# HagesLab/Bayesian-Inference-TRPL

Measured on AMD Instinct MI355X. Metric: TRPL timesteps/sec at 128 nodes (system = parameter sample x excitation; fused solve + log-likelihood; parameter-sample likelihoods/sec in likelihoods_per_s_*), higher is better.
Workload: dtype f64

## Files before the change

### bayesian-inference-trpl_amd/csrc/stepper_pair_impl.hpp

```cpp
#pragma once
#include "stepper_impl.hpp"

namespace trpl {
TRPL_VARIANT_NS_BEGIN
namespace pair {

constexpr int L = 128;
constexpr int NR = 4;
constexpr int WS = 32;

__device__ __forceinline__ double lane_value(double v, int l)
{
    return __hiloint2double(__builtin_amdgcn_readlane(__double2hiint(v), l),
                            __builtin_amdgcn_readlane(__double2loint(v), l));
}

__device__ __forceinline__ void half_sums(double v, double &lo, double &hi)
{
    v = dpp_add<0x111, 0xF>(v);
    v = dpp_add<0x112, 0xF>(v);
    v = dpp_add<0x114, 0xF>(v);
    v = dpp_add<0x118, 0xF>(v);
    v = dpp_add<0x142, 0xA>(v);
    lo = lane_value(v, 31);
    hi = lane_value(v, 63);
}

struct Terms2 {
    double q;
    unsigned long long neg, nonneg;
};
__device__ __forceinline__ Terms2 no_terms2() { return {0.0, 0ull, ~0ull}; }

// ... 39 lines not shown
        }
    }
    if (reductions) (*reductions)++;
    double sA, sB;
    half_sums(t.q, sA, sB);
    okA = sA < 0.0;
    okB = sB < 0.0;
}

template <bool ISO>
__device__ __forceinline__ void update_field2(const MatPar &m, double a0, const double (&Nk)[NR], const double (&Pk)[NR],
                                              const double (&bE)[NR], double (&Ek)[NR], int lane, bool act)
{
    double Nm[NR], Pm[NR], A[NR], b[NR], rA[NR];
    nbrB_dn<double, NR, 1>(Nk, Nm, lane);
    nbrB_dn<double, NR, 1>(Pk, Pm, lane);
    if constexpr (ISO) {
        const bool first = (lane & (WS - 1)) == 0;
        Nm[0] = first ? 0.0 : Nm[0];
        Pm[0] = first ? 0.0 : Pm[0];
    }
#pragma unroll
    for (int j = 0; j < NR; j++) {
        A[j] = __builtin_fma(m.hLDP, Pk[j] + Pm[j], __builtin_fma(m.hLDN, Nk[j] + Nm[j], a0));
        b[j] = __builtin_fma(m.LDP, Pk[j] - Pm[j], __builtin_fma(-m.LDN, Nk[j] - Nm[j], -bE[j]));
    }
    rcp_rows<NR>(A, rA);
    const bool act0 = act && (lane & (WS - 1)) != 0;
    Ek[0] = act0 ? b[0] * rA[0] : Ek[0];
#pragma unroll
    for (int j = 1; j < NR; j++) Ek[j] = act ? b[j] * rA[j] : Ek[j];
}

template <bool ISO, bool SNAP = false, bool OPT = (TRPL_PAIR_OPTIMISTIC != 0)>
__global__ void __launch_bounds__(64, 2) stepper_pair_kernel(const StepArgs a)
{
    constexpr int LAY = 2;
    const int lane = threadIdx.x;
    const int ln = lane & (WS - 1);
    const bool hi = lane >= WS;
    const int64_t blk = blockIdx.x;
    int cA = (int)(blk % a.C), cB = cA;
    int64_t sA = 2 * (blk / a.C), sB = sA + 1;
    if (a.pair_n > 0) {
        const int k = cA;
        cA = a.pair_cA[k]; cB = a.pair_cB[k];
        sB = sA + a.pair_oB[k];
        sA = sA + a.pair_oA[k];
        if (sA >= a.S) return;
    }
    const bool validB = sB < a.S;
    if (!validB) { sB = sA; cB = cA; }
    const int64_t s = hi ? sB : sA;
    const int c = hi ? cB : cA;
    const CurveConst &cc = a.curve[cA];

    const double *xs = a.X + s * a.xld;
    const double N0 = xs[0] * cc.scales[0], P0 = xs[1] * cc.scales[1], DN = xs[2] * cc.scales[2],
                 DP = xs[3] * cc.scales[3], rate = xs[4] * cc.scales[4], sr0 = xs[5] * cc.scales[5],
                 srL = xs[6] * cc.scales[6], CN = xs[7] * cc.scales[7], CP = xs[8] * cc.scales[8],
                 tauN = xs[9] * cc.scales[9], tauP = xs[10] * cc.scales[10],
                 Lambda = xs[11] * cc.scales[11];
    const double n0p0 = N0 * P0;
    MatPar mp_ = {N0, P0, DN, DP, rate, sr0, srL, CN, CP, tauN, tauP, Lambda, n0p0,
                  ln == 0 ? 1.0 : 0.0, ln == WS - 1 ? 1.0 : 0.0};
    mp_.fast_constants();
    mp_.boundary_constants();
    MatPar mp = mp_;
    const double mag = a.xld > 12 ? xs[12] : 0.0;
    const double TOL = a.TOL;
    const int MAX = a.MAX;
    constexpr bool PREDICT = TRPL_STEPPER_PREDICT != 0;

    constexpr int HSLOT = 2 * NR * 64;
    constexpr bool MOMENTS = TRPL_STEPPER_MOMENTS != 0;
    constexpr bool WEIGHTED = TRPL_STEPPER_WEIGHTED != 0;
    constexpr bool CUT = TRPL_STEPPER_CUT != 0;
    constexpr bool PARKED = MOMENTS || CUT;
    static_assert(!CUT || !SNAP, "the cut sink exists in likelihood mode only");
    __shared__ __attribute__((aligned(16))) double lds[4 * HSLOT + (PARKED ? 6 : 0)];
    double2 *hist2 = reinterpret_cast<double2 *>(lds);
    double *xch = nullptr;
    double Nk[NR], Pk[NR], Ek[NR], hE[4][NR];
#pragma unroll
    for (int j = 0; j < NR; j++) {
        const double raw = (SNAP && a.resN != nullptr) ? 0.0 : a.dN[(int64_t)c * L + NR * ln + j];
        const double dn = raw * cc.dx3;
        Nk[j] = N0 + dn;
        Pk[j] = P0 + dn;
        Ek[j] = 0.0;
#pragma unroll
        for (int m = 0; m < 4; m++) {
            hE[m][j] = 0.0;
            hist2[(m * NR + j) * 64 + lane] = make_double2(0.0, 0.0);
        }
    }

    PlSinkT<MOMENTS, PARKED, WEIGHTED, CUT> sinkA(a, cc, cA, sA, lane_value(mag, 0));
    PlSinkT<MOMENTS, PARKED, WEIGHTED, CUT> sinkB(a, cc, cB, sB, lane_value(mag, WS));
    const double rateA = lane_value(rate, 0), rateB = lane_value(rate, WS);
    if constexpr (PARKED) { sinkA.set_park(lds + 4 * HSLOT); sinkB.set_park(lds + 4 * HSLOT + 3); }
    sinkA.set_floor(rateA, lane_value(n0p0, 0), L);
    sinkB.set_floor(rateB, lane_value(n0p0, WS), L);
    int statusA = 0, statusB = 0;
    bool deadA = false, deadB = !validB;
    int64_t itotA = 0, itotB = 0;
#if TRPL_VOTE_STATS
    int nredN = 0, nredP = 0;
#define TRPL_STAT(x) &x
#else
#define TRPL_STAT(x) nullptr
#endif
    SnapSink snap(a, cc);
    auto park = [&](bool mine) {
        if (mine) {
            MatPar b_ = {1.0, 1.0, 1.0, 1.0, 0.0, 0.0, 0.0, 0.0, 0.0, 1.0, 1.0, 0.0, 1.0,
                         ln == 0 ? 1.0 : 0.0, ln == WS - 1 ? 1.0 : 0.0};
            b_.fast_constants();
            b_.boundary_constants();
            mp = b_;
        }
#pragma unroll
        for (int j = 0; j < NR; j++) {
            if (mine) {
                Nk[j] = 1.0; Pk[j] = 1.0; Ek[j] = 0.0;
#pragma unroll
                for (int m = 0; m < 4; m++) {
                    hE[m][j] = 0.0;
                    hist2[(m * NR + j) * 64 + lane] = make_double2(1.0, 1.0);
                }
            }
        }
    };

    int32_t t_begin = 0;
    if constexpr (SNAP) {
        if (a.resN != nullptr) {
            t_begin = (int32_t)a.t0;
            const int64_t r5 = (hi ? sinkB.orow : sinkA.orow) * 5;
#pragma unroll
            for (int j = 0; j < NR; j++) {
                const int i = NR * ln + j;
                Nk[j] = a.resN[(r5 + 4) * L + i]; Pk[j] = a.resP[(r5 + 4) * L + i]; Ek[j] = a.resE[(r5 + 4) * (L + 1) + i];
#pragma unroll
                for (int m = 0; m < 4; m++) {
                    const int slot = (int)((a.t0 - 1 - m) & 3);
                    const double e_ = a.resE[(r5 + 3 - m) * (L + 1) + i];
                    hE[m][j] = e_;
                    hist2[(slot * NR + j) * 64 + lane] = make_double2(a.resN[(r5 + 3 - m) * L + i], a.resP[(r5 + 3 - m) * L + i]);
                }
            }
            statusA = status_of_checkpoint(a.resN[(sinkA.orow * 5 + 4) * L], a.t0);
            statusB = validB ? status_of_checkpoint(a.resN[(sinkB.orow * 5 + 4) * L], a.t0) : 0;
            deadA = statusA != 0;
            deadB = deadB || statusB != 0;
            if (statusA || statusB) park(hi ? statusB != 0 : statusA != 0);
        }
    }
    int32_t pl_next = 0, pl_col = 0;
    if constexpr (SNAP) {
        if (t_begin > 0) { pl_col = (t_begin + a.plT - 1) / a.plT; pl_next = pl_col * a.plT; sinkA.base = sinkB.base = pl_col; }
    }
    const int32_t row_cap = bdf_row_cap(a.flags);
    for (int32_t t = t_begin; t <= sinkA.t_last; t++) {
        if (deadA && deadB) break;
        if constexpr (SNAP) {
            if (snap.due(t))
                snap.template take<NR, L>(Nk, Pk, Ek, hi ? sinkB.orow : sinkA.orow, hi ? !deadB : !deadA,
                                          [&](int j) { return NR * ln + j; });
        }
        double a0, a1, a2, a3, a4, a5;
        bdf_row<double>(t < row_cap ? t : row_cap, a0, a1, a2, a3, a4, a5);

        double plA = 0.0, plB = 0.0;
        const bool pl_step = t == pl_next;
        if (pl_step) {
            double q = __builtin_fma(Nk[0], Pk[0], -n0p0);
#pragma unroll
            for (int j = 1; j < NR; j++) q += __builtin_fma(Nk[j], Pk[j], -n0p0);
            double hA, hB;
            half_sums(q, hA, hB);
            plA = rateA * hA;
            plB = rateB * hB;
        }

        double bN[NR], bP[NR], bE[NR];
        {
            const int s1 = (int)((t + 3) & 3) * NR, s2 = (int)((t + 2) & 3) * NR,
                      s3 = (int)((t + 1) & 3) * NR, s4 = (int)(t & 3) * NR;
#pragma unroll
            for (int j = 0; j < NR; j++) {
                const double2 h1 = hist2[(s1 + j) * 64 + lane], h2 = hist2[(s2 + j) * 64 + lane],
                              h3 = hist2[(s3 + j) * 64 + lane], h4 = hist2[(s4 + j) * 64 + lane];
                bN[j] = a1 * Nk[j] + a2 * h1.x + a3 * h2.x + a4 * h3.x + a5 * h4.x;
                bP[j] = a1 * Pk[j] + a2 * h1.y + a3 * h2.y + a4 * h3.y + a5 * h4.y;
                hist2[(s4 + j) * 64 + lane] = make_double2(Nk[j], Pk[j]);
                if constexpr (PREDICT) {
                    Nk[j] = predict_start(Nk[j], h1.x, h2.x, t);
                    Pk[j] = predict_start(Pk[j], h1.y, h2.y, t);
                }
            }
#pragma unroll
            for (int j = 0; j < NR; j++) {
                bE[j] = a1 * Ek[j] + a2 * hE[0][j] + a3 * hE[1][j] + a4 * hE[2][j] + a5 * hE[3][j];
#pragma unroll
                for (int m = 3; m >= 1; m--) hE[m][j] = hE[m - 1][j];
                hE[0][j] = Ek[j];
                if constexpr (PREDICT) Ek[j] = predict_start(Ek[j], hE[1][j], hE[2][j], t);
            }
        }

        bool doneA = deadA, doneB = deadB;
        int itA = MAX, itB = MAX;
        auto iterate_once = [&](auto frozen_c, auto seam_c, int iters) {
            constexpr bool FROZEN = decltype(frozen_c)::value;
            constexpr bool SEAM = decltype(seam_c)::value;
            const bool act = FROZEN ? (hi ? !doneB : !doneA) : true;
            double lo_[NR], dg[NR], up[NR], bb[NR], Ep[NR], x[NR];
            nbrB_up<double, NR, 1>(Ek, Ep, lane);
            bool okNA, okNB, okPA, okPB;
            const bool needNA = FROZEN ? !doneA : true, needNB = FROZEN ? !doneB : true;
            assemble<LAY, true, NR, WS, L, true>(mp, a0, Nk, Pk, Ek, Ep, bN, lo_, dg, up, bb, ln);
            const Terms2 tN = residual_terms2<SEAM>(lo_, dg, up, bb, Nk, TOL, lane);
            residual_verdict2(tN, needNA, needNB, okNA, okNB, TRPL_STAT(nredN));
            cr_pcr_solve<double, NR, WS, SEAM, true>(lo_, dg, up, bb, x, lane, xch);
#pragma unroll
            for (int j = 0; j < NR; j++) Nk[j] = act ? x[j] : Nk[j];
            assemble<LAY, false, NR, WS, L, true>(mp, a0, Nk, Pk, Ek, Ep, bP, lo_, dg, up, bb, ln);
            const bool needPA = needNA && okNA, needPB = needNB && okNB;
            Terms2 tP = no_terms2();
            if (needPA || needPB) {
                tP = residual_terms2<SEAM>(lo_, dg, up, bb, Pk, TOL, lane);
                residual_verdict2(tP, needPA, needPB, okPA, okPB, TRPL_STAT(nredP));
            } else {
                okPA = okPB = false;
            }
            cr_pcr_solve<double, NR, WS, SEAM, true>(lo_, dg, up, bb, x, lane, xch);
#pragma unroll
            for (int j = 0; j < NR; j++) Pk[j] = act ? x[j] : Pk[j];
            update_field2<ISO>(mp, a0, Nk, Pk, bE, Ek, lane, act);
            if (!doneA && okNA && okPA) { doneA = true; itA = iters + 1; }
            if (!doneB && okNB && okPB) { doneB = true; itB = iters + 1; }
        };
        auto iterate_step = [&](auto seam_c) {
            int iters = 0;
            for (; iters < MAX && !(doneA || doneB); iters++) iterate_once(std::false_type{}, seam_c, iters);
            for (; iters < MAX && !(doneA && doneB); iters++) iterate_once(std::true_type{}, seam_c, iters);
        };
        if constexpr (ISO && OPT) {
            iterate_step(std::false_type{});
            static_assert(NR % 4 == 0, "the witness relies on rcp_rows taking ONE reciprocal of the product of a lane's rows (pcr.hpp)");
            const double wit = Ek[NR - 1];
            const bool finite2 = TRPL_PAIR_WITNESS == 0 || __builtin_amdgcn_ballot_w64(__builtin_isfinite(wit)) == ~0ull;
            if ((!deadA && itA >= MAX) || (!deadB && itB >= MAX) || !finite2) {
                const int s4 = (int)(t & 3) * NR;
#pragma unroll
                for (int j = 0; j < NR; j++) {
                    const double2 h = hist2[(s4 + j) * 64 + lane];
                    if constexpr (PREDICT) {
                        const double2 h1 = hist2[((int)((t + 3) & 3) * NR + j) * 64 + lane],
                                      h2 = hist2[((int)((t + 2) & 3) * NR + j) * 64 + lane];
                        Nk[j] = predict_start(h.x, h1.x, h2.x, t);
                        Pk[j] = predict_start(h.y, h1.y, h2.y, t);
                        Ek[j] = predict_start(hE[0][j], hE[1][j], hE[2][j], t);
                    } else {
                        Nk[j] = h.x; Pk[j] = h.y; Ek[j] = hE[0][j];
                    }
                }
                doneA = deadA; doneB = deadB; itA = itB = MAX;
                iterate_step(std::true_type{});
            }
        } else {
            iterate_step(std::integral_constant<bool, ISO>{});
        }
        bool killA = false, killB = false;
        if (!deadA) { itotA += itA; if (itA >= MAX) { statusA = 1 + (int)t; killA = true; } }
        if (!deadB) { itotB += itB; if (itB >= MAX) { statusB = 1 + (int)t; killB = true; } }
        if (killA || killB) {
            park(hi ? killB : killA);
            deadA = deadA || killA;
            deadB = deadB || killB;
        }

        if (pl_step) {
            if (!deadA) sinkA.push(pl_col, plA);
            if (!deadB) sinkB.push(pl_col, plB);
            pl_next += a.plT;
            pl_col++;
            if constexpr (CUT) {
                if ((pl_col & 63) == 0) {
                    const bool cutA = !deadA && sinkA.is_cut(), cutB = !deadB && sinkB.is_cut();
                    if (cutA || cutB) {
                        park(hi ? cutB : cutA);
                        deadA = deadA || cutA;
                        deadB = deadB || cutB;
                    }
                }
            }
        }

    }

    {
        const int64_t doneA_ = statusA ? (int64_t)(statusA - 1) : sinkA.t_last + 1;
        const int64_t doneB_ = statusB ? (int64_t)(statusB - 1) : sinkB.t_last + 1;
        sinkA.flush_batch((int)((doneA_ + a.plT - 1) / a.plT - sinkA.base));
        if (validB) sinkB.flush_batch((int)((doneB_ + a.plT - 1) / a.plT - sinkB.base));
    }
    if constexpr (SNAP) {
        if (statusA && !hi) snap.template fail_fill<L>(sinkA.orow, statusA, ln, WS);
        if (statusB && hi && validB) snap.template fail_fill<L>(sinkB.orow, statusB, ln, WS);
    }
#if TRPL_VOTE_STATS
    itotA += ((int64_t)nredN << 24) + ((int64_t)nredP << 44);
#endif
    sinkA.finish(statusA, itotA);
    if (validB) sinkB.finish(statusB, itotB);
#undef TRPL_STAT
}

}

template <bool ISO>
hipError_t launch_stepper_pair_t(const StepArgs &a, hipStream_t stream)
{
    if (a.L != pair::L) return hipErrorInvalidValue;
    const int64_t nblk = ((a.S + 1) / 2) * a.C;
    if (nblk <= 0) return hipSuccess;
    const bool always_seam = (a.flags & kFlagPairAlwaysSeam) != 0;
    const bool snap = a.n_snap > 0 || a.resN != nullptr;
    const dim3 grid((unsigned)nblk), block(64);
#if TRPL_STEPPER_MOMENTS || TRPL_STEPPER_CUT
    if (snap || !sink_args_ok(a)) return hipErrorInvalidValue;
    if (always_seam) hipLaunchKernelGGL((pair::stepper_pair_kernel<ISO, false, false>), grid, block, 0, stream, a);
    else             hipLaunchKernelGGL((pair::stepper_pair_kernel<ISO, false>), grid, block, 0, stream, a);
#else
    if (always_seam) {
        if (snap) hipLaunchKernelGGL((pair::stepper_pair_kernel<ISO, true, false>), grid, block, 0, stream, a);
        else      hipLaunchKernelGGL((pair::stepper_pair_kernel<ISO, false, false>), grid, block, 0, stream, a);
    } else {
        if (snap) hipLaunchKernelGGL((pair::stepper_pair_kernel<ISO, true>), grid, block, 0, stream, a);
        else      hipLaunchKernelGGL((pair::stepper_pair_kernel<ISO, false>), grid, block, 0, stream, a);
    }
#endif
    return hipGetLastError();
}
TRPL_VARIANT_NS_END

}
```

### bayesian-inference-trpl_amd/csrc/trpl_api.hip

```cpp
#include <hip/hip_runtime.h>
#include <dlfcn.h>
#include <math.h>
#include <stdarg.h>
#include <stdio.h>
#include <stdlib.h>
#include <string.h>

#include <algorithm>
#include <chrono>
#include <vector>

#include "api_util.hpp"
#include "crosslane.hpp"

namespace trpl {

namespace { thread_local char g_err[512] = ""; }

int api_fail(int code, const char *fmt, ...)
{
    va_list ap;
    va_start(ap, fmt);
    vsnprintf(g_err, sizeof g_err, fmt, ap);
    va_end(ap);
// ... 298 lines not shown

static int no_cut_flag(uint32_t flags)
{
    if (flags & TRPL_FLAG_CUT)
        return api_fail(TRPL_ERR_ARG, "TRPL_FLAG_CUT is set by trpl_loglik_cut[_dev] only: this entry point has no sse_cut");
    return TRPL_OK;
}

int no_weighted_flag(uint32_t flags)
{
    if (int rc = no_cut_flag(flags)) return rc;
    if (flags & TRPL_FLAG_WEIGHTED)
        return api_fail(TRPL_ERR_ARG, "TRPL_FLAG_WEIGHTED is set by trpl_loglik_weighted[_dev] only: this entry point takes no weights");
    return TRPL_OK;
}

int no_moments_flag(uint32_t flags)
{
    if (int rc = no_weighted_flag(flags)) return rc;
    if (flags & TRPL_FLAG_MOMENTS)
        return api_fail(TRPL_ERR_ARG, "TRPL_FLAG_MOMENTS is set by trpl_loglik_moments[_dev] only: this entry point has no esum output");
    return TRPL_OK;
}

int select_device(int32_t device)
{
    int n = 0;
    if (hipGetDeviceCount(&n) != hipSuccess || n <= 0) return api_fail(TRPL_ERR_NODEVICE, "no HIP device visible");
    if (device < 0 || device >= n) return api_fail(TRPL_ERR_ARG, "device %d out of range (%d visible)", device, n);
    HIP_TRY(hipSetDevice(device));
    return TRPL_OK;
}

}

using namespace trpl;

namespace {

int launch(const trpl::StepArgs &a_in, uint32_t flags, hipStream_t st, int64_t steps)
{
    if (int rc = check_launch(flags, a_in.L, steps, a_in.n_snap > 0, a_in.resN != nullptr)) return rc;
    const StepperChoice c = classify_stepper(flags, a_in.L, a_in.S * a_in.C, steps, a_in.n_snap > 0 || a_in.resN != nullptr);
    trpl::StepArgs a = a_in;
    a.bundle = c.bundle;
    if (c.family == StepperChoice::Pair) build_pair_table(a);
    static const char *const kWord[trpl::Variant::kUnits] = {"", "", "pair ", "fp32 ", "mixed ", "hist32 "};
    StepperLauncher *const fn = find_launcher(c);
    if (!fn) return api_fail(TRPL_ERR_UNSUPPORTED, "no stepper is built for this combination of flags (flags 0x%x, L = %d)", flags, a.L);
    const hipError_t e = fn(a, st);
    if (e != hipSuccess) return api_fail(TRPL_ERR_HIP, "%sstepper launch: %s", kWord[unit_of(c)], hipGetErrorString(e));
    return TRPL_OK;
}

}

extern "C" {

int trpl_abi_version(void) { return TRPL_ABI_VERSION; }
int trpl_has_experimental(void)
{
#ifdef TRPL_EXPERIMENTAL
    return 1;
#else
    return 0;
#endif
}
const char *trpl_last_error(void) { return g_err; }

int trpl_kernel_variant(int64_t nsys, int32_t L, int64_t steps, uint32_t flags)
{
    const StepperChoice c = classify_stepper(flags, L, nsys, steps, false);
    if (c.family == StepperChoice::F32) return TRPL_KERNEL_FP32;
    if (c.strict) return TRPL_KERNEL_STRICT;
    if (c.mixed) return TRPL_KERNEL_MIXED;
    if (c.hist32) return TRPL_KERNEL_HIST32;
    return c.family == StepperChoice::Pair ? TRPL_KERNEL_FAST_PAIR : TRPL_KERNEL_FAST;
}

int trpl_kernel_name(int64_t nsys, int32_t L, int64_t steps, uint32_t flags, int32_t snapshots, char *buf, int64_t buflen)
{
    if (!buf || buflen < 1) return api_fail(TRPL_ERR_ARG, "buf must hold at least one byte");
    buf[0] = 0;
    if (int rc = check_launch(flags, L, steps, snapshots != 0 && !(flags & TRPL_FLAG_FP32), false)) return rc;
    const StepperChoice c = classify_stepper(flags, L, nsys, steps, snapshots != 0);
    if (!find_launcher(c)) return api_fail(TRPL_ERR_UNSUPPORTED, "no stepper is built for this combination of flags (flags 0x%x, L = %d)", flags, L);
    const char *tf[2] = {"false", "true"};
    char ns[64];
    snprintf(ns, sizeof ns, "trpl::%s%s", kSinks[c.sink].ns, c.predict ? "predict::" : "");
    int n;
    if (c.family == StepperChoice::F32)
        n = snprintf(buf, (size_t)buflen, "%sf32::stepper_kernel<%d>", ns, c.L);
    else if (c.family == StepperChoice::Pair)
        n = snprintf(buf, (size_t)buflen, "%spair::stepper_pair_kernel<true, %s, %s>", ns, tf[c.snap], tf[c.optimistic]);
    else
        n = snprintf(buf, (size_t)buflen, "%sstepper_kernel<%d, %s, %s, %s, %s, %s>", ns, c.L, tf[c.strict], tf[c.snap],
                     tf[c.mixed], tf[c.bundle > 1], tf[c.hist32]);
    if (n < 0 || n >= buflen) return api_fail(TRPL_ERR_ARG, "buflen=%lld is too small for the kernel name", (long long)buflen);
    return TRPL_OK;
}

// ... 1075 lines not shown
```

### bayesian-inference-trpl_amd/csrc/trpl_common.hpp

```cpp
#pragma once
#include <hip/hip_runtime.h>
#include <stdint.h>

namespace trpl {

constexpr int kMaxCurves = 16;
constexpr int kMaxSnaps = 16;
constexpr int kMaxBundle = 16;
__host__ __device__ constexpr int bundle_cap(int L) { return L <= 64 ? 16 : 4; }

struct CurveConst {
    double scales[12];
    double dx3;
    double plnorm;
    double dx;
    int64_t n_obs;
};

struct StepArgs {
    const double *X;
    const double *dN;
    const double *obs;
    const int32_t *obs_hi;
    const double *obs_dx;
    const double *obs_h;
    void *pl;
    double *sse;
    int32_t *status;
    int64_t *iters_total;
    int32_t *floor_col;
    double *snapN, *snapP, *snapE;
    const double *resN, *resP, *resE;
    int64_t t0;
    int64_t S;
    int64_t T;
    int64_t pl_ld;
    int64_t obs_ld;
    double TOL;
    int32_t xld;
    int32_t C;
    int32_t L;
    int32_t plT;
    int32_t MAX;
    int32_t pl_bytes;
    uint32_t flags;
    int32_t bundle;
    int32_t n_snap;
    int32_t snap_ld;
    int32_t snap_t[kMaxSnaps];
    int32_t snap_slot[kMaxSnaps];
    int32_t pair_n;
    uint8_t pair_cA[kMaxCurves], pair_oA[kMaxCurves], pair_cB[kMaxCurves], pair_oB[kMaxCurves];
    CurveConst curve[kMaxCurves];
    double *esum;
    const double *wts;
    double sse_cut;
    int32_t *cut_col;
    const double *cut_level;
};

__host__ __device__ constexpr uint32_t flags_bdf_order(uint32_t flags) { return (flags >> 14) & 7u; }
__host__ __device__ constexpr int32_t bdf_row_cap(uint32_t flags) { return flags_bdf_order(flags) ? (int32_t)flags_bdf_order(flags) - 1 : 4; }
constexpr int32_t flags_bundle(uint32_t flags) { return (int32_t)((flags >> 8) & 0xFu) + 1; }
template <typename T>
__device__ __forceinline__ void bdf_row(int32_t row, T &a0, T &a1, T &a2, T &a3, T &a4, T &a5)
{
    if (row == 0)      { a0 = (T)1.0; a1 = (T)-1.0; a2 = (T)0.0; a3 = (T)0.0; a4 = (T)0.0; a5 = (T)0.0; }
    else if (row == 1) { a0 = (T)1.5; a1 = (T)-2.0; a2 = (T)0.5; a3 = (T)0.0; a4 = (T)0.0; a5 = (T)0.0; }
    else if (row == 2) { a0 = (T)(11.0 / 6); a1 = (T)-3.0; a2 = (T)1.5; a3 = (T)(-1.0 / 3); a4 = (T)0.0; a5 = (T)0.0; }
    else if (row == 3) { a0 = (T)(25.0 / 12); a1 = (T)-4.0; a2 = (T)3.0; a3 = (T)(-4.0 / 3); a4 = (T)0.25; a5 = (T)0.0; }
    else               { a0 = (T)(137.0 / 60); a1 = (T)-5.0; a2 = (T)5.0; a3 = (T)(-10.0 / 3); a4 = (T)1.25; a5 = (T)-0.2; }
}

void interp_rows_any(const void *pl, int elem_bytes, int64_t rows, int64_t ld, const int32_t *hi, const double *dx,
                     const double *h, int64_t n_obs, double *out, int64_t out_ld);
struct Variant {
    enum Sink { plain, moments, weighted, cut, kSinks };
    enum Unit { fast, strict, pair, f32, mixed, hist32, kUnits };
};
template <int SINK, int PREDICT, int UNIT> hipError_t launch_variant(const StepArgs &a, hipStream_t stream);
#define TRPL_VARIANT(sink, predict, unit) \
    template <> hipError_t launch_variant<Variant::sink, predict, Variant::unit>(const StepArgs &a, hipStream_t stream);
#include "stepper_variants.hpp"
#undef TRPL_VARIANT

hipError_t launch_log10_clamp(void *x, int elem_bytes, int64_t rows, int64_t cols, int64_t ld, double mn,
                              hipStream_t stream);
hipError_t launch_sse_accumulate(double *P, const void *pl, int elem_bytes, int64_t rows, int64_t n_obs,
                                 int64_t ld, const double *values, const double *mag, hipStream_t stream);
hipError_t launch_reduce_curves(double *P, const double *sse, int64_t S, int C, hipStream_t stream);
hipError_t launch_budget_level(const double *budget, const double *sse, double *cut_level, int64_t S, int c0, int g, hipStream_t stream);
hipError_t launch_pl_loglik(const void *pl, int elem_bytes, int64_t rows, int64_t ld, const double *obs,
// ... 39 lines not shown
```

Baseline: 616.4 million.

## Make pair stepper persistent with atomic ticket work distribution

Wraps the pair stepper kernel body in a loop so a resident-sized grid of blocks pulls pair work items from a global atomic ticket counter instead of launching one block per pair. Ticket slots are tracked on the host with events so they can be reused across launches, and a fallback to the classic launch exists when no slot is free. This is meant to balance the uneven per-pair iteration counts and reduce block scheduling tail. The cost is atomic traffic, extra host bookkeeping, and risk around slot reuse and counter reset.

```diff
diff --git a/bayesian-inference-trpl_amd/csrc/stepper_pair_impl.hpp b/bayesian-inference-trpl_amd/csrc/stepper_pair_impl.hpp
--- a/bayesian-inference-trpl_amd/csrc/stepper_pair_impl.hpp
+++ b/bayesian-inference-trpl_amd/csrc/stepper_pair_impl.hpp
@@ -1,4 +1,7 @@
 #pragma once
+#include <atomic>
+#include <mutex>
+
 #include "stepper_impl.hpp"
 
 namespace trpl {
@@ -104,291 +107,405 @@
     for (int j = 1; j < NR; j++) Ek[j] = act ? b[j] * rA[j] : Ek[j];
 }
 
+template <bool SNAP>
+constexpr bool kPersistent = !SNAP && TRPL_STEPPER_PREDICT == 0;
+
+struct Ticket { unsigned next, done; };
+constexpr int kLiveSlots = 32;
+static __device__ Ticket g_ticket[kLiveSlots];
+
 template <bool ISO, bool SNAP = false, bool OPT = (TRPL_PAIR_OPTIMISTIC != 0)>
 __global__ void __launch_bounds__(64, 2) stepper_pair_kernel(const StepArgs a)
 {
-    constexpr int LAY = 2;
-    const int lane = threadIdx.x;
-    const int ln = lane & (WS - 1);
-    const bool hi = lane >= WS;
-    const int64_t blk = blockIdx.x;
-    int cA = (int)(blk % a.C), cB = cA;
-    int64_t sA = 2 * (blk / a.C), sB = sA + 1;
-    if (a.pair_n > 0) {
-        const int k = cA;
-        cA = a.pair_cA[k]; cB = a.pair_cB[k];
-        sB = sA + a.pair_oB[k];
-        sA = sA + a.pair_oA[k];
-        if (sA >= a.S) return;
-    }
-    const bool validB = sB < a.S;
-    if (!validB) { sB = sA; cB = cA; }
-    const int64_t s = hi ? sB : sA;
-    const int c = hi ? cB : cA;
-    const CurveConst &cc = a.curve[cA];
-
-    const double *xs = a.X + s * a.xld;
-    const double N0 = xs[0] * cc.scales[0], P0 = xs[1] * cc.scales[1], DN = xs[2] * cc.scales[2],
-                 DP = xs[3] * cc.scales[3], rate = xs[4] * cc.scales[4], sr0 = xs[5] * cc.scales[5],
-                 srL = xs[6] * cc.scales[6], CN = xs[7] * cc.scales[7], CP = xs[8] * cc.scales[8],
-                 tauN = xs[9] * cc.scales[9], tauP = xs[10] * cc.scales[10],
-                 Lambda = xs[11] * cc.scales[11];
-    const double n0p0 = N0 * P0;
-    MatPar mp_ = {N0, P0, DN, DP, rate, sr0, srL, CN, CP, tauN, tauP, Lambda, n0p0,
-                  ln == 0 ? 1.0 : 0.0, ln == WS - 1 ? 1.0 : 0.0};
-    mp_.fast_constants();
-    mp_.boundary_constants();
-    MatPar mp = mp_;
-    const double mag = a.xld > 12 ? xs[12] : 0.0;
-    const double TOL = a.TOL;
-    const int MAX = a.MAX;
-    constexpr bool PREDICT = TRPL_STEPPER_PREDICT != 0;
-
-    constexpr int HSLOT = 2 * NR * 64;
-    constexpr bool MOMENTS = TRPL_STEPPER_MOMENTS != 0;
-    constexpr bool WEIGHTED = TRPL_STEPPER_WEIGHTED != 0;
-    constexpr bool CUT = TRPL_STEPPER_CUT != 0;
-    constexpr bool PARKED = MOMENTS || CUT;
-    static_assert(!CUT || !SNAP, "the cut sink exists in likelihood mode only");
-    __shared__ __attribute__((aligned(16))) double lds[4 * HSLOT + (PARKED ? 6 : 0)];
-    double2 *hist2 = reinterpret_cast<double2 *>(lds);
-    double *xch = nullptr;
-    double Nk[NR], Pk[NR], Ek[NR], hE[4][NR];
-#pragma unroll
-    for (int j = 0; j < NR; j++) {
-        const double raw = (SNAP && a.resN != nullptr) ? 0.0 : a.dN[(int64_t)c * L + NR * ln + j];
-        const double dn = raw * cc.dx3;
-        Nk[j] = N0 + dn;
-        Pk[j] = P0 + dn;
-        Ek[j] = 0.0;
-#pragma unroll
-        for (int m = 0; m < 4; m++) {
-            hE[m][j] = 0.0;
-            hist2[(m * NR + j) * 64 + lane] = make_double2(0.0, 0.0);
-        }
-    }
-
-    PlSinkT<MOMENTS, PARKED, WEIGHTED, CUT> sinkA(a, cc, cA, sA, lane_value(mag, 0));
-    PlSinkT<MOMENTS, PARKED, WEIGHTED, CUT> sinkB(a, cc, cB, sB, lane_value(mag, WS));
-    const double rateA = lane_value(rate, 0), rateB = lane_value(rate, WS);
-    if constexpr (PARKED) { sinkA.set_park(lds + 4 * HSLOT); sinkB.set_park(lds + 4 * HSLOT + 3); }
-    sinkA.set_floor(rateA, lane_value(n0p0, 0), L);
-    sinkB.set_floor(rateB, lane_value(n0p0, WS), L);
-    int statusA = 0, statusB = 0;
-    bool deadA = false, deadB = !validB;
-    int64_t itotA = 0, itotB = 0;
+    int64_t blk = blockIdx.x;
+    for (;;) {
+#if TRPL_SLOT_TIMELINE
+        const uint64_t t_start = wall_clock64();
+#endif
+        do {
+            constexpr int LAY = 2;
+            int lane_ = threadIdx.x;
+            if constexpr (kPersistent<SNAP>) asm volatile("" : "+v"(lane_));
+            const int lane = lane_;
+            const int ln = lane & (WS - 1);
+            const bool hi = lane >= WS;
+            int cA = (int)(blk % a.C), cB = cA;
+            int64_t sA = 2 * (blk / a.C), sB = sA + 1;
+            if (a.pair_n > 0) {
+                const int k = cA;
+                cA = a.pair_cA[k]; cB = a.pair_cB[k];
+                sB = sA + a.pair_oB[k];
+                sA = sA + a.pair_oA[k];
+                if (sA >= a.S) break;
+            }
+            const bool validB = sB < a.S;
+            if (!validB) { sB = sA; cB = cA; }
+            const int64_t s = hi ? sB : sA;
+            const int c = hi ? cB : cA;
+            const CurveConst &cc = a.curve[cA];
+
+            const double *xs = a.X + s * a.xld;
+            const double N0 = xs[0] * cc.scales[0], P0 = xs[1] * cc.scales[1], DN = xs[2] * cc.scales[2],
+                         DP = xs[3] * cc.scales[3], rate = xs[4] * cc.scales[4], sr0 = xs[5] * cc.scales[5],
+                         srL = xs[6] * cc.scales[6], CN = xs[7] * cc.scales[7], CP = xs[8] * cc.scales[8],
+                         tauN = xs[9] * cc.scales[9], tauP = xs[10] * cc.scales[10],
+                         Lambda = xs[11] * cc.scales[11];
+            const double n0p0 = N0 * P0;
+            MatPar mp_ = {N0, P0, DN, DP, rate, sr0, srL, CN, CP, tauN, tauP, Lambda, n0p0,
+                          ln == 0 ? 1.0 : 0.0, ln == WS - 1 ? 1.0 : 0.0};
+            mp_.fast_constants();
+            mp_.boundary_constants();
+            MatPar mp = mp_;
+            const double mag = a.xld > 12 ? xs[12] : 0.0;
+            const double TOL = a.TOL;
+            const int MAX = a.MAX;
+            constexpr bool PREDICT = TRPL_STEPPER_PREDICT != 0;
+
+            constexpr int HSLOT = 2 * NR * 64;
+            constexpr bool MOMENTS = TRPL_STEPPER_MOMENTS != 0;
+            constexpr bool WEIGHTED = TRPL_STEPPER_WEIGHTED != 0;
+            constexpr bool CUT = TRPL_STEPPER_CUT != 0;
+            constexpr bool PARKED = MOMENTS || CUT;
+            static_assert(!CUT || !SNAP, "the cut sink exists in likelihood mode only");
+            __shared__ __attribute__((aligned(16))) double lds[4 * HSLOT + (PARKED ? 6 : 0)];
+            double2 *hist2 = reinterpret_cast<double2 *>(lds);
+            double *xch = nullptr;
+            double Nk[NR], Pk[NR], Ek[NR], hE[4][NR];
+#pragma unroll
+            for (int j = 0; j < NR; j++) {
+                const double raw = (SNAP && a.resN != nullptr) ? 0.0 : a.dN[(int64_t)c * L + NR * ln + j];
+                const double dn = raw * cc.dx3;
+                Nk[j] = N0 + dn;
+                Pk[j] = P0 + dn;
+                Ek[j] = 0.0;
+#pragma unroll
+                for (int m = 0; m < 4; m++) {
+                    hE[m][j] = 0.0;
+                    hist2[(m * NR + j) * 64 + lane] = make_double2(0.0, 0.0);
+                }
+            }
+
+            PlSinkT<MOMENTS, PARKED, WEIGHTED, CUT> sinkA(a, cc, cA, sA, lane_value(mag, 0));
+            PlSinkT<MOMENTS, PARKED, WEIGHTED, CUT> sinkB(a, cc, cB, sB, lane_value(mag, WS));
+            const double rateA = lane_value(rate, 0), rateB = lane_value(rate, WS);
+            if constexpr (PARKED) { sinkA.set_park(lds + 4 * HSLOT); sinkB.set_park(lds + 4 * HSLOT + 3); }
+            sinkA.set_floor(rateA, lane_value(n0p0, 0), L);
+            sinkB.set_floor(rateB, lane_value(n0p0, WS), L);
+            int statusA = 0, statusB = 0;
+            bool deadA = false, deadB = !validB;
+            int64_t itotA = 0, itotB = 0;
 #if TRPL_VOTE_STATS
-    int nredN = 0, nredP = 0;
+            int nredN = 0, nredP = 0;
 #define TRPL_STAT(x) &x
 #else
 #define TRPL_STAT(x) nullptr
 #endif
-    SnapSink snap(a, cc);
-    auto park = [&](bool mine) {
-        if (mine) {
-            MatPar b_ = {1.0, 1.0, 1.0, 1.0, 0.0, 0.0, 0.0, 0.0, 0.0, 1.0, 1.0, 0.0, 1.0,
-                         ln == 0 ? 1.0 : 0.0, ln == WS - 1 ? 1.0 : 0.0};
-            b_.fast_constants();
-            b_.boundary_constants();
-            mp = b_;
+            SnapSink snap(a, cc);
+            auto park = [&](bool mine) {
+                if (mine) {
+                    MatPar b_ = {1.0, 1.0, 1.0, 1.0, 0.0, 0.0, 0.0, 0.0, 0.0, 1.0, 1.0, 0.0, 1.0,
+                                 ln == 0 ? 1.0 : 0.0, ln == WS - 1 ? 1.0 : 0.0};
+                    b_.fast_constants();
+                    b_.boundary_constants();
+                    mp = b_;
+                }
+#pragma unroll
+                for (int j = 0; j < NR; j++) {
+                    if (mine) {
+                        Nk[j] = 1.0; Pk[j] = 1.0; Ek[j] = 0.0;
+#pragma unroll
+                        for (int m = 0; m < 4; m++) {
+                            hE[m][j] = 0.0;
+                            hist2[(m * NR + j) * 64 + lane] = make_double2(1.0, 1.0);
+                        }
+                    }
+                }
+            };
+
+            int32_t t_begin = 0;
+            if constexpr (SNAP) {
+                if (a.resN != nullptr) {
+                    t_begin = (int32_t)a.t0;
+                    const int64_t r5 = (hi ? sinkB.orow : sinkA.orow) * 5;
+#pragma unroll
+                    for (int j = 0; j < NR; j++) {
+                        const int i = NR * ln + j;
+                        Nk[j] = a.resN[(r5 + 4) * L + i]; Pk[j] = a.resP[(r5 + 4) * L + i]; Ek[j] = a.resE[(r5 + 4) * (L + 1) + i];
+#pragma unroll
+                        for (int m = 0; m < 4; m++) {
+                            const int slot = (int)((a.t0 - 1 - m) & 3);
+                            const double e_ = a.resE[(r5 + 3 - m) * (L + 1) + i];
+                            hE[m][j] = e_;
+                            hist2[(slot * NR + j) * 64 + lane] = make_double2(a.resN[(r5 + 3 - m) * L + i], a.resP[(r5 + 3 - m) * L + i]);
+                        }
+                    }
+                    statusA = status_of_checkpoint(a.resN[(sinkA.orow * 5 + 4) * L], a.t0);
+                    statusB = validB ? status_of_checkpoint(a.resN[(sinkB.orow * 5 + 4) * L], a.t0) : 0;
+                    deadA = statusA != 0;
+                    deadB = deadB || statusB != 0;
+                    if (statusA || statusB) park(hi ? statusB != 0 : statusA != 0);
+                }
+            }
+            int32_t pl_next = 0, pl_col = 0;
+            if constexpr (SNAP) {
+                if (t_begin > 0) { pl_col = (t_begin + a.plT - 1) / a.plT; pl_next = pl_col * a.plT; sinkA.base = sinkB.base = pl_col; }
+            }
+            const int32_t row_cap = bdf_row_cap(a.flags);
+            for (int32_t t = t_begin; t <= sinkA.t_last; t++) {
+                if (deadA && deadB) break;
+                if constexpr (SNAP) {
+                    if (snap.due(t))
+                        snap.template take<NR, L>(Nk, Pk, Ek, hi ? sinkB.orow : sinkA.orow, hi ? !deadB : !deadA,
+                                                  [&](int j) { return NR * ln + j; });
+                }
+                double a0, a1, a2, a3, a4, a5;
+                bdf_row<double>(t < row_cap ? t : row_cap, a0, a1, a2, a3, a4, a5);
+
+                double plA = 0.0, plB = 0.0;
+                const bool pl_step = t == pl_next;
+                if (pl_step) {
+                    double q = __builtin_fma(Nk[0], Pk[0], -n0p0);
+#pragma unroll
+                    for (int j = 1; j < NR; j++) q += __builtin_fma(Nk[j], Pk[j], -n0p0);
+                    double hA, hB;
+                    half_sums(q, hA, hB);
+                    plA = rateA * hA;
+                    plB = rateB * hB;
+                }
+
+                double bN[NR], bP[NR], bE[NR];
+                {
+                    const int s1 = (int)((t + 3) & 3) * NR, s2 = (int)((t + 2) & 3) * NR,
+                              s3 = (int)((t + 1) & 3) * NR, s4 = (int)(t & 3) * NR;
+#pragma unroll
+                    for (int j = 0; j < NR; j++) {
+                        const double2 h1 = hist2[(s1 + j) * 64 + lane], h2 = hist2[(s2 + j) * 64 + lane],
+                                      h3 = hist2[(s3 + j) * 64 + lane], h4 = hist2[(s4 + j) * 64 + lane];
+                        bN[j] = a1 * Nk[j] + a2 * h1.x + a3 * h2.x + a4 * h3.x + a5 * h4.x;
+                        bP[j] = a1 * Pk[j] + a2 * h1.y + a3 * h2.y + a4 * h3.y + a5 * h4.y;
+                        hist2[(s4 + j) * 64 + lane] = make_double2(Nk[j], Pk[j]);
+                        if constexpr (PREDICT) {
+                            Nk[j] = predict_start(Nk[j], h1.x, h2.x, t);
+                            Pk[j] = predict_start(Pk[j], h1.y, h2.y, t);
+                        }
+                    }
+#pragma unroll
+                    for (int j = 0; j < NR; j++) {
+                        bE[j] = a1 * Ek[j] + a2 * hE[0][j] + a3 * hE[1][j] + a4 * hE[2][j] + a5 * hE[3][j];
+#pragma unroll
+                        for (int m = 3; m >= 1; m--) hE[m][j] = hE[m - 1][j];
+                        hE[0][j] = Ek[j];
+                        if constexpr (PREDICT) Ek[j] = predict_start(Ek[j], hE[1][j], hE[2][j], t);
+                    }
+                }
+
+                bool doneA = deadA, doneB = deadB;
+                int itA = MAX, itB = MAX;
+                auto iterate_once = [&](auto frozen_c, auto seam_c, int iters) {
+                    constexpr bool FROZEN = decltype(frozen_c)::value;
+                    constexpr bool SEAM = decltype(seam_c)::value;
+                    const bool act = FROZEN ? (hi ? !doneB : !doneA) : true;
+                    double lo_[NR], dg[NR], up[NR], bb[NR], Ep[NR], x[NR];
+                    nbrB_up<double, NR, 1>(Ek, Ep, lane);
+                    bool okNA, okNB, okPA, okPB;
+                    const bool needNA = FROZEN ? !doneA : true, needNB = FROZEN ? !doneB : true;
+                    assemble<LAY, true, NR, WS, L, true>(mp, a0, Nk, Pk, Ek, Ep, bN, lo_, dg, up, bb, ln);
+                    const Terms2 tN = residual_terms2<SEAM>(lo_, dg, up, bb, Nk, TOL, lane);
+                    residual_verdict2(tN, needNA, needNB, okNA, okNB, TRPL_STAT(nredN));
+                    cr_pcr_solve<double, NR, WS, SEAM, true>(lo_, dg, up, bb, x, lane, xch);
+#pragma unroll
+                    for (int j = 0; j < NR; j++) Nk[j] = act ? x[j] : Nk[j];
+                    assemble<LAY, false, NR, WS, L, true>(mp, a0, Nk, Pk, Ek, Ep, bP, lo_, dg, up, bb, ln);
+                    const bool needPA = needNA && okNA, needPB = needNB && okNB;
+                    Terms2 tP = no_terms2();
+                    if (needPA || needPB) {
+                        tP = residual_terms2<SEAM>(lo_, dg, up, bb, Pk, TOL, lane);
+                        residual_verdict2(tP, needPA, needPB, okPA, okPB, TRPL_STAT(nredP));
+                    } else {
+                        okPA = okPB = false;
+                    }
+                    cr_pcr_solve<double, NR, WS, SEAM, true>(lo_, dg, up, bb, x, lane, xch);
+#pragma unroll
+                    for (int j = 0; j < NR; j++) Pk[j] = act ? x[j] : Pk[j];
+                    update_field2<ISO>(mp, a0, Nk, Pk, bE, Ek, lane, act);
+                    if (!doneA && okNA && okPA) { doneA = true; itA = iters + 1; }
+                    if (!doneB && okNB && okPB) { doneB = true; itB = iters + 1; }
+                };
+                auto iterate_step = [&](auto seam_c) {
+                    int iters = 0;
+                    for (; iters < MAX && !(doneA || doneB); iters++) iterate_once(std::false_type{}, seam_c, iters);
+                    for (; iters < MAX && !(doneA && doneB); iters++) iterate_once(std::true_type{}, seam_c, iters);
+                };
+                if constexpr (ISO && OPT) {
+                    iterate_step(std::false_type{});
+                    static_assert(NR % 4 == 0, "the witness relies on rcp_rows taking ONE reciprocal of the product of a lane's rows (pcr.hpp)");
+                    const double wit = Ek[NR - 1];
+                    const bool finite2 = TRPL_PAIR_WITNESS == 0 || __builtin_amdgcn_ballot_w64(__builtin_isfinite(wit)) == ~0ull;
+                    if ((!deadA && itA >= MAX) || (!deadB && itB >= MAX) || !finite2) {
+                        const int s4 = (int)(t & 3) * NR;
+#pragma unroll
+                        for (int j = 0; j < NR; j++) {
+                            const double2 h = hist2[(s4 + j) * 64 + lane];
+                            if constexpr (PREDICT) {
+                                const double2 h1 = hist2[((int)((t + 3) & 3) * NR + j) * 64 + lane],
+                                              h2 = hist2[((int)((t + 2) & 3) * NR + j) * 64 + lane];
+                                Nk[j] = predict_start(h.x, h1.x, h2.x, t);
+                                Pk[j] = predict_start(h.y, h1.y, h2.y, t);
+                                Ek[j] = predict_start(hE[0][j], hE[1][j], hE[2][j], t);
+                            } else {
+                                Nk[j] = h.x; Pk[j] = h.y; Ek[j] = hE[0][j];
+                            }
+                        }
+                        doneA = deadA; doneB = deadB; itA = itB = MAX;
+                        iterate_step(std::true_type{});
+                    }
+                } else {
+                    iterate_step(std::integral_constant<bool, ISO>{});
+                }
+                bool killA = false, killB = false;
+                if (!deadA) { itotA += itA; if (itA >= MAX) { statusA = 1 + (int)t; killA = true; } }
+                if (!deadB) { itotB += itB; if (itB >= MAX) { statusB = 1 + (int)t; killB = true; } }
+                if (killA || killB) {
+                    park(hi ? killB : killA);
+                    deadA = deadA || killA;
+                    deadB = deadB || killB;
+                }
+
+                if (pl_step) {
+                    if (!deadA) sinkA.push(pl_col, plA);
+                    if (!deadB) sinkB.push(pl_col, plB);
+                    pl_next += a.plT;
+                    pl_col++;
+                    if constexpr (CUT) {
+                        if ((pl_col & 63) == 0) {
+                            const bool cutA = !deadA && sinkA.is_cut(), cutB = !deadB && sinkB.is_cut();
+                            if (cutA || cutB) {
+                                park(hi ? cutB : cutA);
+                                deadA = deadA || cutA;
+                                deadB = deadB || cutB;
+                            }
+                        }
+                    }
+                }
+
+            }
+
+            {
+                const int64_t doneA_ = statusA ? (int64_t)(statusA - 1) : sinkA.t_last + 1;
+                const int64_t doneB_ = statusB ? (int64_t)(statusB - 1) : sinkB.t_last + 1;
+                sinkA.flush_batch((int)((doneA_ + a.plT - 1) / a.plT - sinkA.base));
+                if (validB) sinkB.flush_batch((int)((doneB_ + a.plT - 1) / a.plT - sinkB.base));
+            }
+            if constexpr (SNAP) {
+                if (statusA && !hi) snap.template fail_fill<L>(sinkA.orow, statusA, ln, WS);
+                if (statusB && hi && validB) snap.template fail_fill<L>(sinkB.orow, statusB, ln, WS);
+            }
+#if TRPL_VOTE_STATS
+            itotA += ((int64_t)nredN << 24) + ((int64_t)nredP << 44);
+#endif
+            sinkA.finish(statusA, itotA);
+            if (validB) sinkB.finish(statusB, itotB);
+#undef TRPL_STAT
+        } while (false);
+#if TRPL_SLOT_TIMELINE
+        if (a.timeline != nullptr && threadIdx.x == 0) {
+            const uint64_t hw = (uint32_t)__builtin_amdgcn_s_getreg(4 | (31 << 11));
+            const uint64_t xcc = (uint32_t)__builtin_amdgcn_s_getreg(20 | (31 << 11));
+            uint64_t *rec = a.timeline + 4 * blk;
+            rec[0] = (uint64_t)blk; rec[1] = t_start; rec[2] = wall_clock64(); rec[3] = hw | (xcc << 32);
         }
-#pragma unroll
-        for (int j = 0; j < NR; j++) {
-            if (mine) {
-                Nk[j] = 1.0; Pk[j] = 1.0; Ek[j] = 0.0;
-#pragma unroll
-                for (int m = 0; m < 4; m++) {
-                    hE[m][j] = 0.0;
-                    hist2[(m * NR + j) * 64 + lane] = make_double2(1.0, 1.0);
-                }
-            }
+#endif
+        if (!kPersistent<SNAP> || a.ticket_slot < 0) return;
+        const int64_t nblk = ((a.S + 1) / 2) * a.C;
+        const unsigned grid = gridDim.x;
+        Ticket *const tk = &g_ticket[a.ticket_slot];
+        unsigned drawn = 0;
+        if (threadIdx.x == 0) drawn = atomicAdd(&tk->next, 1u);
+        blk = (int64_t)grid + (unsigned)__builtin_amdgcn_readfirstlane((int)drawn);
+        if (blk >= nblk) {
+            if (threadIdx.x == 0 && atomicAdd(&tk->done, 1u) == grid - 1) {
+                atomicExch(&tk->next, 0u);
+                atomicExch(&tk->done, 0u);
+            }
+            return;
         }
-    };
-
-    int32_t t_begin = 0;
-    if constexpr (SNAP) {
-        if (a.resN != nullptr) {
-            t_begin = (int32_t)a.t0;
-            const int64_t r5 = (hi ? sinkB.orow : sinkA.orow) * 5;
-#pragma unroll
-            for (int j = 0; j < NR; j++) {
-                const int i = NR * ln + j;
-                Nk[j] = a.resN[(r5 + 4) * L + i]; Pk[j] = a.resP[(r5 + 4) * L + i]; Ek[j] = a.resE[(r5 + 4) * (L + 1) + i];
-#pragma unroll
-                for (int m = 0; m < 4; m++) {
-                    const int slot = (int)((a.t0 - 1 - m) & 3);
-                    const double e_ = a.resE[(r5 + 3 - m) * (L + 1) + i];
-                    hE[m][j] = e_;
-                    hist2[(slot * NR + j) * 64 + lane] = make_double2(a.resN[(r5 + 3 - m) * L + i], a.resP[(r5 + 3 - m) * L + i]);
-                }
-            }
-            statusA = status_of_checkpoint(a.resN[(sinkA.orow * 5 + 4) * L], a.t0);
-            statusB = validB ? status_of_checkpoint(a.resN[(sinkB.orow * 5 + 4) * L], a.t0) : 0;
-            deadA = statusA != 0;
-            deadB = deadB || statusB != 0;
-            if (statusA || statusB) park(hi ? statusB != 0 : statusA != 0);
+    }
+}
+
+constexpr int kMaxDevices = 64;
+template <typename Kern>
+int resident_waves(Kern kern, int dev)
+{
+    static std::atomic<int> cache[kMaxDevices];
+    int r = cache[dev].load(std::memory_order_relaxed);
+    if (r > 0) return r;
+    int cus = 0, per_cu = 0;
+    if (hipDeviceGetAttribute(&cus, hipDeviceAttributeMultiprocessorCount, dev) != hipSuccess ||
+        hipOccupancyMaxActiveBlocksPerMultiprocessor(&per_cu, kern, 64, 0) != hipSuccess || cus < 1 || per_cu < 1) {
+        (void)hipGetLastError();
+        return 0;
+    }
+    r = cus * per_cu;
+    cache[dev].store(r, std::memory_order_relaxed);
+    return r;
+}
+
+struct TicketHost {
+    std::mutex mu;
+    hipEvent_t ev[kLiveSlots] = {};
+    bool made[kLiveSlots] = {}, busy[kLiveSlots] = {}, retired[kLiveSlots] = {};
+};
+static TicketHost g_ticket_host[kMaxDevices];
+
+template <bool SNAP, typename Kern>
+hipError_t launch_pair_blocks(Kern kern, StepArgs a, int64_t nblk, hipStream_t stream)
+{
+    a.ticket_slot = -1;
+    int dev = -1;
+    if (hipGetDevice(&dev) != hipSuccess) return hipGetLastError();
+    const int resident = kPersistent<SNAP> && dev < kMaxDevices ? resident_waves(kern, dev) : 0;
+    bool persistent = resident > 0 && nblk > resident;
+#if TRPL_SLOT_TIMELINE
+    if (a.timeline_classic) persistent = false;
+#endif
+    if (resident > 0) g_pair_launch_info[2].store(resident, std::memory_order_relaxed);
+    if (!persistent) {
+        g_pair_launch_info[1].fetch_add(1, std::memory_order_relaxed);
+        hipLaunchKernelGGL(kern, dim3((unsigned)nblk), dim3(64), 0, stream, a);
+        return hipGetLastError();
+    }
+    hipStreamCaptureStatus cap = hipStreamCaptureStatusNone;
+    if (hipStreamIsCapturing(stream, &cap) != hipSuccess) { (void)hipGetLastError(); cap = hipStreamCaptureStatusInvalidated; }
+    TicketHost &h = g_ticket_host[dev];
+    std::lock_guard<std::mutex> lock(h.mu);
+    int slot = -1;
+    if (cap == hipStreamCaptureStatusNone) {
+        for (int i = 0; i < kLiveSlots && slot < 0; i++) {
+            if (h.retired[i]) continue;
+            if (!h.made[i]) {
+                if (hipEventCreateWithFlags(&h.ev[i], hipEventDisableTiming) != hipSuccess) { (void)hipGetLastError(); h.retired[i] = true; continue; }
+                h.made[i] = true;
+            }
+            if (h.busy[i]) {
+                const hipError_t q = hipEventQuery(h.ev[i]);
+                if (q != hipSuccess) { (void)hipGetLastError(); continue; }
+                h.busy[i] = false;
+            }
+            slot = i;
         }
     }
-    int32_t pl_next = 0, pl_col = 0;
-    if constexpr (SNAP) {
-        if (t_begin > 0) { pl_col = (t_begin + a.plT - 1) / a.plT; pl_next = pl_col * a.plT; sinkA.base = sinkB.base = pl_col; }
-    }
-    const int32_t row_cap = bdf_row_cap(a.flags);
-    for (int32_t t = t_begin; t <= sinkA.t_last; t++) {
-        if (deadA && deadB) break;
-        if constexpr (SNAP) {
-            if (snap.due(t))
-                snap.template take<NR, L>(Nk, Pk, Ek, hi ? sinkB.orow : sinkA.orow, hi ? !deadB : !deadA,
-                                          [&](int j) { return NR * ln + j; });
-        }
-        double a0, a1, a2, a3, a4, a5;
-        bdf_row<double>(t < row_cap ? t : row_cap, a0, a1, a2, a3, a4, a5);
-
-        double plA = 0.0, plB = 0.0;
-        const bool pl_step = t == pl_next;
-        if (pl_step) {
-            double q = __builtin_fma(Nk[0], Pk[0], -n0p0);
-#pragma unroll
-            for (int j = 1; j < NR; j++) q += __builtin_fma(Nk[j], Pk[j], -n0p0);
-            double hA, hB;
-            half_sums(q, hA, hB);
-            plA = rateA * hA;
-            plB = rateB * hB;
-        }
-
-        double bN[NR], bP[NR], bE[NR];
-        {
-            const int s1 = (int)((t + 3) & 3) * NR, s2 = (int)((t + 2) & 3) * NR,
-                      s3 = (int)((t + 1) & 3) * NR, s4 = (int)(t & 3) * NR;
-#pragma unroll
-            for (int j = 0; j < NR; j++) {
-                const double2 h1 = hist2[(s1 + j) * 64 + lane], h2 = hist2[(s2 + j) * 64 + lane],
-                              h3 = hist2[(s3 + j) * 64 + lane], h4 = hist2[(s4 + j) * 64 + lane];
-                bN[j] = a1 * Nk[j] + a2 * h1.x + a3 * h2.x + a4 * h3.x + a5 * h4.x;
-                bP[j] = a1 * Pk[j] + a2 * h1.y + a3 * h2.y + a4 * h3.y + a5 * h4.y;
-                hist2[(s4 + j) * 64 + lane] = make_double2(Nk[j], Pk[j]);
-                if constexpr (PREDICT) {
-                    Nk[j] = predict_start(Nk[j], h1.x, h2.x, t);
-                    Pk[j] = predict_start(Pk[j], h1.y, h2.y, t);
-                }
-            }
-#pragma unroll
-            for (int j = 0; j < NR; j++) {
-                bE[j] = a1 * Ek[j] + a2 * hE[0][j] + a3 * hE[1][j] + a4 * hE[2][j] + a5 * hE[3][j];
-#pragma unroll
-                for (int m = 3; m >= 1; m--) hE[m][j] = hE[m - 1][j];
-                hE[0][j] = Ek[j];
-                if constexpr (PREDICT) Ek[j] = predict_start(Ek[j], hE[1][j], hE[2][j], t);
-            }
-        }
-
-        bool doneA = deadA, doneB = deadB;
-        int itA = MAX, itB = MAX;
-        auto iterate_once = [&](auto frozen_c, auto seam_c, int iters) {
-            constexpr bool FROZEN = decltype(frozen_c)::value;
-            constexpr bool SEAM = decltype(seam_c)::value;
-            const bool act = FROZEN ? (hi ? !doneB : !doneA) : true;
-            double lo_[NR], dg[NR], up[NR], bb[NR], Ep[NR], x[NR];
-            nbrB_up<double, NR, 1>(Ek, Ep, lane);
-            bool okNA, okNB, okPA, okPB;
-            const bool needNA = FROZEN ? !doneA : true, needNB = FROZEN ? !doneB : true;
-            assemble<LAY, true, NR, WS, L, true>(mp, a0, Nk, Pk, Ek, Ep, bN, lo_, dg, up, bb, ln);
-            const Terms2 tN = residual_terms2<SEAM>(lo_, dg, up, bb, Nk, TOL, lane);
-            residual_verdict2(tN, needNA, needNB, okNA, okNB, TRPL_STAT(nredN));
-            cr_pcr_solve<double, NR, WS, SEAM, true>(lo_, dg, up, bb, x, lane, xch);
-#pragma unroll
-            for (int j = 0; j < NR; j++) Nk[j] = act ? x[j] : Nk[j];
-            assemble<LAY, false, NR, WS, L, true>(mp, a0, Nk, Pk, Ek, Ep, bP, lo_, dg, up, bb, ln);
-            const bool needPA = needNA && okNA, needPB = needNB && okNB;
-            Terms2 tP = no_terms2();
-            if (needPA || needPB) {
-                tP = residual_terms2<SEAM>(lo_, dg, up, bb, Pk, TOL, lane);
-                residual_verdict2(tP, needPA, needPB, okPA, okPB, TRPL_STAT(nredP));
-            } else {
-                okPA = okPB = false;
-            }
-            cr_pcr_solve<double, NR, WS, SEAM, true>(lo_, dg, up, bb, x, lane, xch);
-#pragma unroll
-            for (int j = 0; j < NR; j++) Pk[j] = act ? x[j] : Pk[j];
-            update_field2<ISO>(mp, a0, Nk, Pk, bE, Ek, lane, act);
-            if (!doneA && okNA && okPA) { doneA = true; itA = iters + 1; }
-            if (!doneB && okNB && okPB) { doneB = true; itB = iters + 1; }
-        };
-        auto iterate_step = [&](auto seam_c) {
-            int iters = 0;
-            for (; iters < MAX && !(doneA || doneB); iters++) iterate_once(std::false_type{}, seam_c, iters);
-            for (; iters < MAX && !(doneA && doneB); iters++) iterate_once(std::true_type{}, seam_c, iters);
-        };
-        if constexpr (ISO && OPT) {
-            iterate_step(std::false_type{});
-            static_assert(NR % 4 == 0, "the witness relies on rcp_rows taking ONE reciprocal of the product of a lane's rows (pcr.hpp)");
-            const double wit = Ek[NR - 1];
-            const bool finite2 = TRPL_PAIR_WITNESS == 0 || __builtin_amdgcn_ballot_w64(__builtin_isfinite(wit)) == ~0ull;
-            if ((!deadA && itA >= MAX) || (!deadB && itB >= MAX) || !finite2) {
-                const int s4 = (int)(t & 3) * NR;
-#pragma unroll
-                for (int j = 0; j < NR; j++) {
-                    const double2 h = hist2[(s4 + j) * 64 + lane];
-                    if constexpr (PREDICT) {
-                        const double2 h1 = hist2[((int)((t + 3) & 3) * NR + j) * 64 + lane],
-                                      h2 = hist2[((int)((t + 2) & 3) * NR + j) * 64 + lane];
-                        Nk[j] = predict_start(h.x, h1.x, h2.x, t);
-                        Pk[j] = predict_start(h.y, h1.y, h2.y, t);
-                        Ek[j] = predict_start(hE[0][j], hE[1][j], hE[2][j], t);
-                    } else {
-                        Nk[j] = h.x; Pk[j] = h.y; Ek[j] = hE[0][j];
-                    }
-                }
-                doneA = deadA; doneB = deadB; itA = itB = MAX;
-                iterate_step(std::true_type{});
-            }
-        } else {
-            iterate_step(std::integral_constant<bool, ISO>{});
-        }
-        bool killA = false, killB = false;
-        if (!deadA) { itotA += itA; if (itA >= MAX) { statusA = 1 + (int)t; killA = true; } }
-        if (!deadB) { itotB += itB; if (itB >= MAX) { statusB = 1 + (int)t; killB = true; } }
-        if (killA || killB) {
-            park(hi ? killB : killA);
-            deadA = deadA || killA;
-            deadB = deadB || killB;
-        }
-
-        if (pl_step) {
-            if (!deadA) sinkA.push(pl_col, plA);
-            if (!deadB) sinkB.push(pl_col, plB);
-            pl_next += a.plT;
-            pl_col++;
-            if constexpr (CUT) {
-                if ((pl_col & 63) == 0) {
-                    const bool cutA = !deadA && sinkA.is_cut(), cutB = !deadB && sinkB.is_cut();
-                    if (cutA || cutB) {
-                        park(hi ? cutB : cutA);
-                        deadA = deadA || cutA;
-                        deadB = deadB || cutB;
-                    }
-                }
-            }
-        }
-
-    }
-
-    {
-        const int64_t doneA_ = statusA ? (int64_t)(statusA - 1) : sinkA.t_last + 1;
-        const int64_t doneB_ = statusB ? (int64_t)(statusB - 1) : sinkB.t_last + 1;
-        sinkA.flush_batch((int)((doneA_ + a.plT - 1) / a.plT - sinkA.base));
-        if (validB) sinkB.flush_batch((int)((doneB_ + a.plT - 1) / a.plT - sinkB.base));
-    }
-    if constexpr (SNAP) {
-        if (statusA && !hi) snap.template fail_fill<L>(sinkA.orow, statusA, ln, WS);
-        if (statusB && hi && validB) snap.template fail_fill<L>(sinkB.orow, statusB, ln, WS);
-    }
-#if TRPL_VOTE_STATS
-    itotA += ((int64_t)nredN << 24) + ((int64_t)nredP << 44);
-#endif
-    sinkA.finish(statusA, itotA);
-    if (validB) sinkB.finish(statusB, itotB);
-#undef TRPL_STAT
+    if (slot < 0) {
+        g_pair_launch_info[1].fetch_add(1, std::memory_order_relaxed);
+        hipLaunchKernelGGL(kern, dim3((unsigned)nblk), dim3(64), 0, stream, a);
+        return hipGetLastError();
+    }
+    g_pair_launch_info[0].fetch_add(1, std::memory_order_relaxed);
+    a.ticket_slot = slot;
+    hipLaunchKernelGGL(kern, dim3((unsigned)resident), dim3(64), 0, stream, a);
+    const hipError_t e = hipGetLastError();
+    if (hipEventRecord(h.ev[slot], stream) == hipSuccess) h.busy[slot] = true;
+    else { (void)hipGetLastError(); h.retired[slot] = true; }
+    return e;
 }
 
 }
@@ -401,21 +518,18 @@
     if (nblk <= 0) return hipSuccess;
     const bool always_seam = (a.flags & kFlagPairAlwaysSeam) != 0;
     const bool snap = a.n_snap > 0 || a.resN != nullptr;
-    const dim3 grid((unsigned)nblk), block(64);
 #if TRPL_STEPPER_MOMENTS || TRPL_STEPPER_CUT
     if (snap || !sink_args_ok(a)) return hipErrorInvalidValue;
-    if (always_seam) hipLaunchKernelGGL((pair::stepper_pair_kernel<ISO, false, false>), grid, block, 0, stream, a);
-    else             hipLaunchKernelGGL((pair::stepper_pair_kernel<ISO, false>), grid, block, 0, stream, a);
+    if (always_seam) return pair::launch_pair_blocks<false>(pair::stepper_pair_kernel<ISO, false, false>, a, nblk, stream);
+    return pair::launch_pair_blocks<false>(pair::stepper_pair_kernel<ISO, false>, a, nblk, stream);
 #else
     if (always_seam) {
-        if (snap) hipLaunchKernelGGL((pair::stepper_pair_kernel<ISO, true, false>), grid, block, 0, stream, a);
-        else      hipLaunchKernelGGL((pair::stepper_pair_kernel<ISO, false, false>), grid, block, 0, stream, a);
-    } else {
-        if (snap) hipLaunchKernelGGL((pair::stepper_pair_kernel<ISO, true>), grid, block, 0, stream, a);
-        else      hipLaunchKernelGGL((pair::stepper_pair_kernel<ISO, false>), grid, block, 0, stream, a);
-    }
+        if (snap) return pair::launch_pair_blocks<true>(pair::stepper_pair_kernel<ISO, true, false>, a, nblk, stream);
+        return pair::launch_pair_blocks<false>(pair::stepper_pair_kernel<ISO, false, false>, a, nblk, stream);
+    }
+    if (snap) return pair::launch_pair_blocks<true>(pair::stepper_pair_kernel<ISO, true>, a, nblk, stream);
+    return pair::launch_pair_blocks<false>(pair::stepper_pair_kernel<ISO, false>, a, nblk, stream);
 #endif
-    return hipGetLastError();
 }
 TRPL_VARIANT_NS_END
 
diff --git a/bayesian-inference-trpl_amd/csrc/trpl_api.hip b/bayesian-inference-trpl_amd/csrc/trpl_api.hip
--- a/bayesian-inference-trpl_amd/csrc/trpl_api.hip
+++ b/bayesian-inference-trpl_amd/csrc/trpl_api.hip
@@ -354,11 +354,18 @@
     return TRPL_OK;
 }
 
+std::atomic<int64_t> g_pair_launch_info[3];
+
 }
 
 using namespace trpl;
 
 namespace {
+
+#if TRPL_SLOT_TIMELINE
+uint64_t *g_slot_timeline = nullptr;
+int32_t g_slot_timeline_classic = 0;
+#endif
 
 int launch(const trpl::StepArgs &a_in, uint32_t flags, hipStream_t st, int64_t steps)
 {
@@ -367,6 +374,9 @@
     trpl::StepArgs a = a_in;
     a.bundle = c.bundle;
     if (c.family == StepperChoice::Pair) build_pair_table(a);
+#if TRPL_SLOT_TIMELINE
+    a.timeline = g_slot_timeline; a.timeline_classic = g_slot_timeline_classic;
+#endif
     static const char *const kWord[trpl::Variant::kUnits] = {"", "", "pair ", "fp32 ", "mixed ", "hist32 "};
     StepperLauncher *const fn = find_launcher(c);
     if (!fn) return api_fail(TRPL_ERR_UNSUPPORTED, "no stepper is built for this combination of flags (flags 0x%x, L = %d)", flags, a.L);
@@ -389,6 +399,15 @@
 #endif
 }
 const char *trpl_last_error(void) { return g_err; }
+
+void trpl_pair_launch_info(int64_t *out)
+{
+    for (int i = 0; i < 3; i++) out[i] = trpl::g_pair_launch_info[i].load(std::memory_order_relaxed);
+}
+
+#if TRPL_SLOT_TIMELINE
+void trpl_debug_slot_timeline(void *buf, int32_t classic) { g_slot_timeline = (uint64_t *)buf; g_slot_timeline_classic = classic; }
+#endif
 
 int trpl_kernel_variant(int64_t nsys, int32_t L, int64_t steps, uint32_t flags)
 {
diff --git a/bayesian-inference-trpl_amd/csrc/trpl_common.hpp b/bayesian-inference-trpl_amd/csrc/trpl_common.hpp
--- a/bayesian-inference-trpl_amd/csrc/trpl_common.hpp
+++ b/bayesian-inference-trpl_amd/csrc/trpl_common.hpp
@@ -1,6 +1,12 @@
 #pragma once
 #include <hip/hip_runtime.h>
 #include <stdint.h>
+
+#include <atomic>
+
+#ifndef TRPL_SLOT_TIMELINE
+#define TRPL_SLOT_TIMELINE 0
+#endif
 
 namespace trpl {
 
@@ -57,7 +63,14 @@
     double sse_cut;
     int32_t *cut_col;
     const double *cut_level;
+    int32_t ticket_slot;
+#if TRPL_SLOT_TIMELINE
+    uint64_t *timeline;
+    int32_t timeline_classic;
+#endif
 };
+
+extern std::atomic<int64_t> g_pair_launch_info[3];
 
 __host__ __device__ constexpr uint32_t flags_bdf_order(uint32_t flags) { return (flags >> 14) & 7u; }
 __host__ __device__ constexpr int32_t bdf_row_cap(uint32_t flags) { return flags_bdf_order(flags) ? (int32_t)flags_bdf_order(flags) - 1 : 4; }
```

Result: faster. 628.6 million, median of 6 (+2.0%).
